# johannah/drqv2

Measured on AMD Instinct MI355X. Metric: agent updates/sec (batch=256, 9x84x84 obs), higher is better.
Workload: dtype f32; 1 GPU; cheetah_run batch_size=256/GPU (256 global) 9x84x84 u8 obs, A=6, feature_dim=50, hidden_dim=1024, fp32, use_tb=True; parallelism=dp1, global_batch=256

## Files before the change

drqv2_amd/_lib.py:

```python
import ctypes as C
import os

HERE = os.path.dirname(os.path.abspath(__file__))
LIB_PATH = os.path.join(HERE, "libdrqv2_hip.so")

c_float_p = C.c_void_p
c_u8_p = C.c_void_p
stream_t = C.c_void_p


class DrqStep(C.Structure):
    _fields_ = [
        ("B", C.c_int), ("global_B", C.c_int), ("C", C.c_int), ("A", C.c_int), ("F", C.c_int), ("H", C.c_int),
        ("obs", c_u8_p), ("next_obs", c_u8_p),
        ("action", c_float_p), ("reward", c_float_p), ("discount", c_float_p),
        ("shift_obs", c_float_p), ("shift_next", c_float_p),
        ("noise_critic", c_float_p), ("noise_actor", c_float_p),
        ("base_grid", c_float_p),
        ("params", c_float_p), ("grads", c_float_p), ("adam_m", c_float_p), ("adam_v", c_float_p),
        ("ws", c_float_p), ("ws_bytes", C.c_size_t),
        ("sums", c_float_p),
        ("lr", C.c_double), ("tau", C.c_double),
        ("std", C.c_float), ("clip", C.c_float),
        ("step_critic", C.c_long), ("step_enc", C.c_long), ("step_actor", C.c_long),
# ... 11 lines not shown

I, L, F, D, P, SZ = C.c_int, C.c_long, C.c_float, C.c_double, C.c_void_p, C.c_size_t

PROTOTYPES = {
    "drq_abi_version": (I, []),
    "drq_aug_fwd": (I, [P, P, P, P, I, I, I, I, I, P]),
    "drq_aug_fwd_f32": (I, [P, P, P, P, I, I, I, I, P]),
    "drq_conv1_aug_fwd": (I, [P, P, P, P, P, P, P, P, P, I, I, P]),
    "drq_conv1_aug_fwd_bf16": (I, [P, P, P, P, P, P, P, P, P, I, I, P]),
    "drq_conv1_aug_fwd_bf16_nhwc": (I, [P, P, P, P, P, P, P, P, P, I, I, P]),
    "drq_conv1_aug_fwd_indexed": (I, [P, P, P, P, P, P, P, P, P, P, P, I, I, P]),
    "drq_conv3x3_fwd": (I, [P, P, P, P, I, I, I, I, I, L, L, L, L, P]),
    "drq_conv3x3_dgrad": (I, [P, P, P, P, I, I, L, L, L, L, P]),
    "drq_conv3x3_fwd_wino": (I, [P, P, P, P, I, I, I, L, L, L, L, P]),
    "drq_conv3x3_dgrad_wino": (I, [P, P, P, P, I, I, L, L, L, L, P]),
    "drq_conv3x3_wgrad_wino": (I, [P, P, P, P, I, I, L, L, L, L, P, SZ, P]),
    "drq_conv3x3_wgrad": (I, [P, P, P, P, I, I, I, I, L, L, L, L, P, SZ, P]),
    "drq_conv3x3_wgrad_ws_bytes": (SZ, []),
    "drq_conv3x3_fwd_bf16": (I, [P, P, P, P, I, I, I, L, L, L, L, P]),
    "drq_conv3x3_dgrad_bf16": (I, [P, P, P, P, I, I, L, L, L, L, P]),
    "drq_conv3x3_wgrad_bf16": (I, [P, P, P, P, I, I, L, L, L, L, P, SZ, P]),
    "drq_conv3x3_fwd_bf16_nhwc": (I, [P, P, P, P, I, I, I, I, I, P]),
    "drq_conv3x3_dgrad_bf16_nhwc": (I, [P, P, P, P, I, I, I, I, L, L, L, L, P]),
    "drq_conv3x3_wgrad_bf16_nhwc": (I, [P, P, P, P, I, I, I, L, L, L, L, P, SZ, P]),
    "drq_gemm_f32": (I, [P, L, I, P, L, I, P, L, I, I, I, I, L, L, L, P, L, I, P, I, L, I, I, I, P, SZ, P]),
    "drq_gemm_batched_f32": (I, [I, P, L, I, P, L, I, P, L, I, I, I, P, I, P, I, P, I, I, I, P, SZ, P]),
    "drq_gemm_batched_bf16": (I, [I, P, L, I, P, L, I, P, L, I, I, I, P, I, P, I, P, I, I, P, SZ, P]),
    "drq_gemm_batched_partial": (I, [I, P, L, I, P, L, I, P, L, I, I, I, P, P, SZ, C.POINTER(I), P]),
    "drq_mlp_fwd": (I, [I, P, L, P, L, P, L, I, I, I, P, I, P, P, C.POINTER(I), P]),
    "drq_mlp_dgrad": (I, [I, P, L, P, L, P, L, I, I, I, P, I, P]),
# ... 29 lines not shown
    "drq_aug_bwd_f32": (I, [P, P, P, P, I, I, I, I, P]),
    "drq_tanh_bwd": (I, [P, P, P, L, P]),
    "drq_param_layout": (I, [I, I, I, I, C.POINTER(L), I]),
    "drq_step_ws_bytes": (SZ, [I, I, I, I, I]),
    "drq_step_ws_offset": (L, [I, I, I, I, I, I]),
    "drq_update_phase": (I, [C.POINTER(DrqStep), I]),
    "drq_update_phase_bc": (I, [C.POINTER(DrqStep), I, F]),
    "drq_act_forward": (I, [C.POINTER(DrqStep), P, I, P]),
    "drq_act_ws_bytes": (SZ, [I, I, I, I, I]),
    "drq_act_batch": (I, [P, I, I, I, I, P, I, P, F, P, P, P, SZ, P]),
    "drq_publish_sums": (I, [P, P, C.c_uint, P]),
    "drq_rng_draws": (I, [C.c_uint64, C.c_uint64, I, I, I, P, P, P, P, P]),
}

WS_IDS = ["AUG", "ACT1", "ACT2", "ACT3", "FEAT", "Z_NEXT", "Z_OBS", "HA_T", "HA_C", "H_AN", "H_AO", "Q", "TQ",
          "DQ", "MU_O", "DY4", "DY3", "DY2", "DY1", "DZ_C", "DZ_A", "HA_C2", "P1", "P2", "C1", "C2"]

PHASE_ALL, PHASE_CRITIC, PHASE_ACTOR, PHASE_OPT = -1, 0, 1, 2
PHASE_ENCODE, PHASE_CRITIC_HEADS, PHASE_CONV_BACKWARD, PHASE_ACTOR_FORWARD, PHASE_ACTOR_BACKWARD = 3, 4, 5, 6, 7
PHASE_ENCODER_OPT, PHASE_ACTOR_OPT = 8, 9
PHASE_CRITIC_OPT, PHASE_ACTOR_LOSS, PHASE_POLYAK, PHASE_REDRAW = 10, 11, 12, 13

_lib = None


class DrqError(RuntimeError):
    pass


def load():
    global _lib
# ... 41 lines not shown
```

drqv2_amd/csrc/conv_wino.hip:

```cpp
#include "common.h"
#include "internal.h"
#include "wino_u.h"
#include <type_traits>

namespace {

struct WinoArgs {
  const float* x;
  const float* w;
  const float* pre;
  const float* bias;
  const float* mask;
  float* y;
  int y_bs, y_cs, y_rs, y_off;
  unsigned x_bytes, y_bytes, mask_bytes;
  int nb;
  int relu;
  int wmode;
  int stagger;
};

typedef unsigned u32x4w __attribute__((ext_vector_type(4)));
typedef unsigned u32x2w __attribute__((ext_vector_type(2)));
typedef float f32x2w __attribute__((ext_vector_type(2)));

constexpr int kStagger = 0;

template <int HIN, bool MASK, bool RELU>
__global__ __launch_bounds__(256, 2) void conv3x3_wino_kernel(WinoArgs a) {
#pragma clang fp contract(off)
  constexpr int HOUT = HIN - 2;
  constexpr int TH = (HOUT + 1) / 2;
  constexpr int TT = TH * TH;
  constexpr int PLANE = HIN * HIN * 4;
  __shared__ __attribute__((aligned(16))) float U[16 * 8 * 64 * 2];

  const int tid = threadIdx.x;
  const int lane = tid & 63;
  const int wid = tid >> 6;
  const int tl = lane & 15;
  const int kk = lane >> 4;

  if (a.pre) {
// ... 12 lines not shown
  for (int h = 0; h < 2; ++h)
#pragma unroll
    for (int r = 0; r < 4; ++r) bv[h][r] = a.bias ? a.bias[16 * h + 4 * kk + r] : 0.f;
  __syncthreads();

  if (a.stagger) {
    const unsigned hwid = __builtin_amdgcn_s_getreg((4 << 0) | (0 << 6) | (31 << 11));
    if (hwid & 1u)
      for (int q = 0; q < a.stagger; ++q) __builtin_amdgcn_s_sleep(16);
  }

  const __amdgpu_buffer_rsrc_t xrs = __builtin_amdgcn_make_buffer_rsrc((void*)a.x, 0, a.x_bytes, 0x00020000);
  const __amdgpu_buffer_rsrc_t yrs = __builtin_amdgcn_make_buffer_rsrc((void*)a.y, 0, a.y_bytes, 0x00020000);
  const __amdgpu_buffer_rsrc_t mrs =
      __builtin_amdgcn_make_buffer_rsrc((void*)a.mask, 0, a.mask ? a.mask_bytes : 0, 0x00020000);
  constexpr int kDrop = (int)0x80000000u;

  const int ntile = a.nb * TT;
  const int nunit = (ntile + 15) >> 4;
  const int nwave = (int)gridDim.x * 4;
  const f32x2w* Ul = reinterpret_cast<const f32x2w*>(U) + lane;

  auto patch_voff = [&](int unit) {
    int t = unit * 16 + tl;
    t = t < ntile ? t : ntile - 1;
    const int b = t / TT, rem = t - b * TT;
    const int ty = rem / TH, tx = rem - ty * TH;
    return (((b * 32 + kk) * HIN + 2 * ty) * HIN + 2 * tx) * 4;
  };
  auto load_patch_row = [&](float (&d)[16], int voff, int c, int i) {
// ... 50 lines not shown
    const int t = valid ? t0 : ntile - 1;
    const int b = t / TT, rem = t - b * TT;
    const int ty = rem / TH, tx = rem - ty * TH;
    const bool c1ok = 2 * tx + 1 < HOUT, r1ok = 2 * ty + 1 < HOUT;
    const int ybase = (a.y_off + b * a.y_bs + (4 * kk) * a.y_cs + (2 * ty) * a.y_rs + 2 * tx) * 4;
    const int mbase = (((b * 32 + 4 * kk) * HOUT + 2 * ty) * HOUT + 2 * tx) * 4;
    int o64[2], o32[2];
#pragma unroll
    for (int i = 0; i < 2; ++i) {
      const bool rowok = valid && (i == 0 || r1ok);
      o64[i] = (rowok && c1ok) ? ybase : kDrop;
      o32[i] = (rowok && !c1ok) ? ybase : kDrop;
    }
    f32x4 acc[16][2];
    u32x2w mk[2][4][2];
#pragma unroll
    for (int c = 0; c < 8; ++c) {
      asm volatile("" ::: "memory");
      float t[16];
#pragma unroll
      for (int j = 0; j < 4; ++j) {
        t[0 * 4 + j] = d[0 * 4 + j] - d[2 * 4 + j];
        t[1 * 4 + j] = d[1 * 4 + j] + d[2 * 4 + j];
        t[2 * 4 + j] = d[2 * 4 + j] - d[1 * 4 + j];
        t[3 * 4 + j] = d[1 * 4 + j] - d[3 * 4 + j];
      }
      __builtin_amdgcn_sched_barrier(0);
      load_A(A1, c, 1);
      __builtin_amdgcn_sched_barrier(0);
      float V[16];
// ... 16 lines not shown
          const f32x2w Ap = A[p];
          if (c == 0) {
            const f32x4 z = {0.f, 0.f, 0.f, 0.f};
            const f32x4 b0 = {bv[0][0], bv[0][1], bv[0][2], bv[0][3]}, b1 = {bv[1][0], bv[1][1], bv[1][2], bv[1][3]};
            if constexpr (HSEL != 1) acc[pos][0] = __builtin_amdgcn_mfma_f32_16x16x4f32(Ap[0], V[pos], pos == 5 ? b0 : z, 0, 0, 0);
            if constexpr (HSEL != 0) acc[pos][1] = __builtin_amdgcn_mfma_f32_16x16x4f32(Ap[1], V[pos], pos == 5 ? b1 : z, 0, 0, 0);
          } else {
            if constexpr (HSEL != 1) acc[pos][0] = __builtin_amdgcn_mfma_f32_16x16x4f32(Ap[0], V[pos], acc[pos][0], 0, 0, 0);
            if constexpr (HSEL != 0) acc[pos][1] = __builtin_amdgcn_mfma_f32_16x16x4f32(Ap[1], V[pos], acc[pos][1], 0, 0, 0);
          }
        }
      };
      half_step(A0, 0);
      __builtin_amdgcn_sched_barrier(0);
      load_A(A0, (c + 1) & 7, 0);
      if constexpr (MASK) {
        if (c == 7) {
          constexpr int h0 = HSEL == 1 ? 1 : 0;
#pragma unroll
          for (int r = 0; r < 4; ++r)
#pragma unroll
            for (int i = 0; i < 2; ++i)
              mk[h0][r][i] = __builtin_amdgcn_raw_buffer_load_b64(mrs, mbase + i * (HOUT * 4),
                                                                  (16 * h0 + r) * (HOUT * HOUT * 4), 0);
        }
      }
      __builtin_amdgcn_sched_barrier(0);
      half_step(A1, 1);
      __builtin_amdgcn_sched_barrier(0);
    }
    {
      if constexpr (MASK && HSEL == 2) {
#pragma unroll
        for (int r = 0; r < 4; ++r)
#pragma unroll
          for (int i = 0; i < 2; ++i)
            mk[1][r][i] = __builtin_amdgcn_raw_buffer_load_b64(mrs, mbase + i * (HOUT * 4), (16 + r) * (HOUT * HOUT * 4), 0);
        __builtin_amdgcn_sched_barrier(0);
      }
      const int ycs4 = a.y_cs * 4, yrs4 = a.y_rs * 4;
#pragma unroll
      for (int h = (HSEL == 1 ? 1 : 0); h < (HSEL == 0 ? 1 : 2); ++h)
#pragma unroll
        for (int r = 0; r < 4; ++r) {
          float s[2][4];
#pragma unroll
          for (int j = 0; j < 4; ++j) {
            const float m0 = acc[0 * 4 + j][h][r], m1 = acc[1 * 4 + j][h][r], m2 = acc[2 * 4 + j][h][r],
                        m3 = acc[3 * 4 + j][h][r];
            s[0][j] = (m0 + m1) + m2;
            s[1][j] = (m1 - m2) - m3;
          }
          const int co = (16 * h + r);
#pragma unroll
          for (int i = 0; i < 2; ++i) {
            float y0 = (s[i][0] + s[i][1]) + s[i][2];
            float y1 = (s[i][1] - s[i][2]) - s[i][3];
            if constexpr (RELU) {
              y0 = __builtin_fmaxf(y0, 0.f);
              y1 = __builtin_fmaxf(y1, 0.f);
            }
            if constexpr (MASK) {
              const unsigned q0 = mk[h][r][i][0], q1 = mk[h][r][i][1];
              y0 = __uint_as_float(q0) > 0.f ? y0 : 0.f;
              y1 = __uint_as_float(q1) > 0.f ? y1 : 0.f;
            }
            const int soff = co * ycs4 + i * yrs4;
            const u32x2w pk = {__float_as_uint(y0), __float_as_uint(y1)};
            __builtin_amdgcn_raw_buffer_store_b64(pk, yrs, o64[i], soff, 0);
            __builtin_amdgcn_raw_buffer_store_b32(__float_as_uint(y0), yrs, o32[i], soff, 0);
          }
        }
    }
    voff = nvoff;
  };
  for (int i = 0; i < nfull; ++i) body(std::integral_constant<int, 2>{}, item_unit(i), item_unit(i + 1 < nitem ? i + 1 : i));
  if (has_half) {
    if (half_h == 0) body(std::integral_constant<int, 0>{}, half_unit, half_unit);
    else body(std::integral_constant<int, 1>{}, half_unit, half_unit);
  }
}

template <int HIN>
int launch_wino(const WinoArgs& a0, hipStream_t st) {
  WinoArgs a = a0;
  a.stagger = kStagger;
  constexpr int HOUT = HIN - 2, TH = (HOUT + 1) / 2;
  const long nunit = ((long)a.nb * TH * TH + 15) / 16;
  long blocks = (nunit + 3) / 4;
  const long cap = 2L * drq_num_cus();
  if (blocks > cap) blocks = cap;
  if (blocks < 1) blocks = 1;
  const dim3 g((unsigned)blocks), t(256);
  if (a.mask && a.relu) hipLaunchKernelGGL((conv3x3_wino_kernel<HIN, true, true>), g, t, 0, st, a);
  else if (a.mask) hipLaunchKernelGGL((conv3x3_wino_kernel<HIN, true, false>), g, t, 0, st, a);
  else if (a.relu) hipLaunchKernelGGL((conv3x3_wino_kernel<HIN, false, true>), g, t, 0, st, a);
  else hipLaunchKernelGGL((conv3x3_wino_kernel<HIN, false, false>), g, t, 0, st, a);
  DRQ_LAUNCH_CHECK();
  return DRQ_OK;
}

}

int drq_conv3x3_fwd_wino_pre(const float* x, const float* w, const float* u_image, const float* bias, float* y, int nb,
                             int hin, int relu, long y_bs, long y_cs, long y_rs, long y_off, hipStream_t st) {
  if (!x || !w || !y || nb <= 0) return DRQ_EARG;
  const size_t xb = (size_t)nb * 32 * hin * hin * 4;
  const size_t yb = (size_t)nb * y_bs * 4;
  if (xb >= (1ull << 31) || yb >= (1ull << 31) || y_off < 0 || y_bs <= 0) return DRQ_EARG;
  WinoArgs a{x, w, u_image, bias, nullptr, y, (int)y_bs, (int)y_cs, (int)y_rs, (int)y_off, (unsigned)xb, (unsigned)yb, 0u, nb, relu, 0, 0};
  if (hin == 41) return launch_wino<41>(a, st);
  if (hin == 39) return launch_wino<39>(a, st);
  if (hin == 37) return launch_wino<37>(a, st);
  return DRQ_EARG;
}

int drq_conv3x3_dgrad_wino_pre(const float* dy_pad, const float* w, const float* u_image, const float* mask, float* dx,
                               int nb, int hout, long dx_bs, long dx_cs, long dx_rs, long dx_off, hipStream_t st) {
  if (!dy_pad || !w || !dx || nb <= 0) return DRQ_EARG;
  const int hp = hout + 4;
  const size_t xb = (size_t)nb * 32 * hp * hp * 4;
  const size_t yb = (size_t)nb * dx_bs * 4;
  const size_t mb = (size_t)nb * 32 * (hout + 2) * (hout + 2) * 4;
  if (xb >= (1ull << 31) || yb >= (1ull << 31) || dx_off < 0 || dx_bs <= 0) return DRQ_EARG;
  WinoArgs a{dy_pad, w, u_image, nullptr, mask, dx, (int)dx_bs, (int)dx_cs, (int)dx_rs, (int)dx_off, (unsigned)xb, (unsigned)yb,
             (unsigned)mb, nb, 0, 1, 0};
  if (hp == 39) return launch_wino<39>(a, st);
  if (hp == 41) return launch_wino<41>(a, st);
  if (hp == 43) return launch_wino<43>(a, st);
  return DRQ_EARG;
}

DRQ_API int drq_conv3x3_fwd_wino(const float* x, const float* w, const float* bias, float* y, int nb, int hin, int relu,
                                 long y_bs, long y_cs, long y_rs, long y_off, hipStream_t st) {
  return drq_conv3x3_fwd_wino_pre(x, w, nullptr, bias, y, nb, hin, relu, y_bs, y_cs, y_rs, y_off, st);
}

DRQ_API int drq_conv3x3_dgrad_wino(const float* dy_pad, const float* w, const float* mask, float* dx, int nb, int hout,
                                   long dx_bs, long dx_cs, long dx_rs, long dx_off, hipStream_t st) {
  return drq_conv3x3_dgrad_wino_pre(dy_pad, w, nullptr, mask, dx, nb, hout, dx_bs, dx_cs, dx_rs, dx_off, st);
}
```

drqv2_amd/csrc/internal.h:

```cpp
#pragma once
#include "common.h"

int drq_ln_tanh_fwd_multi_ex(int n, const float* const* z, int ldz, const float* const* gamma,
                             const float* const* beta, float* const* out, const int* ldo, float* const* xhat,
                             float* const* rstd, int rows, int F, const float* const* tail, const int* tail_ld,
                             int tail_n, hipStream_t st);
int drq_ln_tanh_fwd_multi_part(int n, const float* const* z, int ldz, const float* const* gamma,
                               const float* const* beta, float* const* out, const int* ldo, float* const* xhat,
                               float* const* rstd, int rows, int F, const float* const* tail, const int* tail_ld,
                               int tail_n, const float* part, const float* const* bias, int splitk, hipStream_t st);
int drq_ln_tanh_bwd_part(const float* dh0, int ld0, const float* dh1, int ld1, const float* h, int ldh,
                         const float* xhat, const float* rstd, const float* gamma, float* dz, float* dln,
                         float* dgamma, float* dbeta, int rows, int F, const float* part, int splitk, int nprob,
                         int ldp, hipStream_t st);
int drq_ln_param_grad(const float* dln, const float* xhat, float* dgamma, float* dbeta, int rows, int F,
                      hipStream_t st);
int drq_qout_bwd_td(const float* tq1, const float* tq2, const float* q1, const float* q2, const float* reward,
                    const float* discount, float inv_global_B, float* sums, const float* const* h,
                    const float* const* w, float* const* dh, float* const* dw, float* const* db, int B, int H,
                    hipStream_t st);
int drq_qout_bwd_actor(const float* q1, const float* q2, const float* act, long lda, const float* mu, float std, int A,
                       float inv_global_B, float* sums, float* sums_host, unsigned seq, const float* const* h,
                       const float* const* w, float* const* dh, int B, int H, hipStream_t st);
int drq_policy_out_fwd(const float* h2, const float* w, const float* b, float* p3, int rows, int H, int A,
// ... 50 lines not shown
int drq_lnl1_fwd(int njobs, const float* const* part, const float* const* z, const float* const* bias,
                 const float* const* gamma, const float* const* beta, float* const* out, const int* ldo,
                 float* const* xhat, float* const* rstd, const float* const* tail, const int* tail_ld, const int* tail_n,
                 const int* rows, const int* nheads, const float* const* w, const float* const* b, float* const* y, int F,
                 int H, int splitk, long slab, hipStream_t st);
int drq_polout_l1_fwd(const float* p2, const float* w3, const float* b3, float* p3, int rows, int srow0, int H, int A,
                      int F, float std, float clip, int use_clip, const float* noise_hi, float* mu_hi, float* ha_hi,
                      long lda_hi, const float* noise_lo, float* mu_lo, float* ha_lo, long lda_lo, int nheads,
                      const float* const* w, const float* const* b, float* const* y, hipStream_t st);

int drq_conv1_aug_fwd_any(int bf_mma, const uint8_t* obs, const float* shift, const uint8_t* obs1, const float* shift1,
                          const float* base_grid, const float* w, const float* bias, float* xaug, float* y, int n,
                          int n_store, hipStream_t st, const float* const* wino_w, float* wino_u, const long* fidx0,
                          const long* fidx1);

int drq_conv3x3_fwd_wino_pre(const float* x, const float* w, const float* u_image, const float* bias, float* y, int nb,
                             int hin, int relu, long y_bs, long y_cs, long y_rs, long y_off, hipStream_t st);
int drq_conv3x3_dgrad_wino_pre(const float* dy_pad, const float* w, const float* u_image, const float* mask, float* dx,
                               int nb, int hout, long dx_bs, long dx_cs, long dx_rs, long dx_off, hipStream_t st);

int drq_conv3x3_fwd_bf16_lay(const void* x, const float* w, const float* bias, void* y, int nb, int hin, int relu,
                             long y_bs, long y_cs, long y_rs, long y_off, int lay, hipStream_t st);
int drq_conv3x3_dgrad_bf16_lay(const void* dy_pad, const float* w, const void* mask, void* dx, int nb, int hout,
                               long dx_bs, long dx_cs, long dx_rs, long dx_off, int lay, hipStream_t st);
int drq_conv3x3_wgrad_partial_bf16_lay(const void* x, const void* dy, int nb, int hin, long dy_bs, long dy_cs, long dy_rs,
                                       long dy_off, float* part, size_t part_bytes, int* nblocks, int lay,
                                       hipStream_t st);
int drq_conv3x3_wgrad_partial_bf16(const float* x, const float* dy, int nb, int hin, long dy_bs, long dy_cs, long dy_rs,
                                   long dy_off, float* part, size_t part_bytes, int* nblocks, hipStream_t st);

constexpr int kActMaxRows = 256;
struct ActWeights {
  const float *enc_w[4], *enc_b[4];
  const float *trunk_w, *trunk_b, *ln_g, *ln_b;
// ... 19 lines not shown
```

drqv2_amd/csrc/step.hip:

```cpp
#include "common.h"
#include "internal.h"
#include "../../include/drqv2_hip.h"

namespace {

constexpr long R = 32L * 35 * 35;
inline long al64(long x) { return (x + 63) & ~63L; }
inline long al512(long x) { return (x + 511) & ~511L; }

struct HeadOff {
  long trunk_w, trunk_b, ln_g, ln_b;
  long w[2][3], b[2][3];
};
enum { SEG_ENC, SEG_CRITIC, SEG_ACTOR, SEG_TARGET };
struct ParamLayout {
  long enc_w[4], enc_b[4];
  HeadOff critic, actor, target;
  long seg[8];
  long total;
  long flat[50];
  int nflat;
  long seg_beg(int net) const { return seg[2 * net]; }
  long seg_len(int net) const { return seg[2 * net + 1] - seg[2 * net]; }
};
// ... 47 lines not shown
}

struct WsLayout {
  long off[64];
  long total;
};
constexpr long kGemmWsFloats = 16L * 1024 * 1024;
enum {
  W_AUG = DRQ_WS_AUG, W_ACT1 = DRQ_WS_ACT1, W_ACT2 = DRQ_WS_ACT2, W_ACT3 = DRQ_WS_ACT3, W_FEAT = DRQ_WS_FEAT,
  W_Z_NEXT = DRQ_WS_Z_NEXT, W_Z_OBS = DRQ_WS_Z_OBS, W_HA_T = DRQ_WS_HA_T, W_HA_C = DRQ_WS_HA_C,
  W_H_AN = DRQ_WS_H_AN, W_H_AO = DRQ_WS_H_AO, W_Q = DRQ_WS_Q, W_TQ = DRQ_WS_TQ, W_DQ = DRQ_WS_DQ,
  W_MU_O = DRQ_WS_MU_O, W_DY4 = DRQ_WS_DY4, W_DY3 = DRQ_WS_DY3, W_DY2 = DRQ_WS_DY2, W_DY1 = DRQ_WS_DY1,
  W_DZ_C = DRQ_WS_DZ_C, W_DZ_A = DRQ_WS_DZ_A, W_HA_C2 = DRQ_WS_HA_C2,
  W_P1 = DRQ_WS_P1, W_P2 = DRQ_WS_P2,
  W_C1 = DRQ_WS_C1, W_C2 = DRQ_WS_C2,
  W_XHAT_C = DRQ_WS_NBUF_PUBLIC, W_RSTD_C, W_XHAT_A, W_RSTD_A, W_Z_C2,
  W_HROWS, W_P3, W_Z4,
  W_T1, W_T2,
  W_DC2, W_DC1, W_DHA, W_DLN, W_DPRE, W_DP2, W_DP1, W_DH_A, W_DA,
  W_GEMM_WS, W_CONV_WS,
  W_WINO_U,
  W_COUNT
};

WsLayout ws_layout(int B, int C, int A, int F, int H) {
  WsLayout w{};
  long off = 0;
  auto take = [&](int id, long n) {
    w.off[id] = off;
    off = al64(off + n);
// ... 35 lines not shown
  take(W_T2, 2L * B * H);
  take(W_C1, 2L * B * H);
  take(W_C2, 2L * B * H);
  take(W_DC2, 2L * B * H);
  take(W_DC1, 2L * B * H);
  take(W_DHA, 2L * B * (F + A));
  take(W_DLN, (long)B * F);
  take(W_DPRE, (long)B * A);
  take(W_DP2, (long)B * H);
  take(W_DP1, (long)B * H);
  take(W_DH_A, (long)B * F);
  take(W_DA, 2L * B * A);
  take(W_GEMM_WS, kGemmWsFloats);
  take(W_CONV_WS, (long)(drq_conv3x3_wgrad_ws_bytes() / sizeof(float)));
  take(W_WINO_U, 6L * 16384);
  w.total = off;
  return w;
}

#define CK(expr)                \
  do {                          \
    const int rc__ = (expr);    \
    if (rc__ != 0) return rc__; \
  } while (0)

struct Ctx {
  const DrqStep* s;
  ParamLayout P;
  WsLayout W;
  hipStream_t st;
  bool fuse_actor_loss = false;
  float bc_alpha = 0.f;
  bool bc() const { return bc_alpha > 0.f; }
  const float* a_beh() const { return ws(W_HA_C) + s->F; }
  float bc_scale() const { return 2.0f / ((float)s->global_B * (float)s->A); }
  bool qout_loss_fits_lds() const { return ((size_t)s->B + 5 * 1024 + 16) * 4 <= 60 * 1024; }
  bool actor_loss_fused() const { return fuse_actor_loss && qout_loss_fits_lds(); }
  bool fuse_rows() const {
    return !(s->flags & DRQ_STEP_NO_ROW_FUSION) && !s->bf16 && s->A <= 32 && s->F + s->A <= 64 && s->F % 2 == 0 &&
           s->A % 2 == 0 && s->H % 256 == 0;
  }
  bool use_gemm3() const { return !(s->flags & DRQ_STEP_NO_GEMM3) && !s->bf16; }
  int stamp(int idx) const {
    if (s->timing_events && idx < s->timing_n && hipEventRecord((hipEvent_t)s->timing_events[idx], st) != hipSuccess)
      return DRQ_EARG;
    return 0;
  }
  float* ws(int id) const { return s->ws + W.off[id]; }
  float* p(long off) const { return s->params + off; }
  float* g(long off) const { return s->grads + off; }
  int bf16() const { return s->bf16 ? 1 : 0; }
  bool acts16() const { return s->bf16 && !(s->flags & DRQ_STEP_BF16_FP32_ACTS); }
  bool grads16() const { return acts16() && !(s->flags & DRQ_STEP_BF16_FP32_GRADS); }
  int adam_segment(int net, long step, int target = -1) const {
    const long o = P.seg_beg(net);
    return drq_adam_flat(p(o), g(o), s->adam_m + o, s->adam_v + o, P.seg_len(net), s->lr, step, s->gscale,
                         target >= 0 ? p(P.seg_beg(target)) : nullptr, target >= 0 ? s->tau : 0.0, st);
// ... 41 lines not shown
    if (use_gemm3() && n >= 2) {
      const int rc = drq_gemm3_wgrad_dgrad(n, dy, lddy, x, ldx, dw, db, w, ldw, dx, lddx, mask, ldmask, Brows, N, K, st);
      if (rc != DRQ_EARG) return rc;
    }
    if (!bf16()) {
      const int rc = drq_gemm2_wgrad_dgrad(n, dy, lddy, x, ldx, dw, db, w, ldw, dx, lddx, mask, ldmask, Brows, N, K, st);
      if (rc != DRQ_EARG) return rc;
    }
    const int rc = wgrad(n, dy, lddy, x, ldx, dw, db, Brows, N, K);
    if (rc != 0) return rc;
    return dgrad(n, dy, lddy, w, ldw, dx, lddx, Brows, K, N, mask, ldmask);
  }
};

int encoder_forward(const Ctx& c, const float* x, int nb, float* a1, float* a2, float* a3, float* a4,
                    bool timed = false) {
  const ParamLayout& P = c.P;
  float* outs[4] = {a1, a2, a3, a4};
  const float* in = x ? x : a1;
  for (int l = x ? 0 : 1; l < 4; ++l) {
    const int hin = kEncH[l], hout = kEncH[l + 1];
    if (timed && l == 1) CK(c.stamp(0));
    if (c.bf16() && l > 0)
      CK(drq_conv3x3_fwd_bf16_lay(in, c.p(P.enc_w[l]), c.p(P.enc_b[l]), outs[l], nb, hin, 1, 32L * hout * hout,
                                  (long)hout * hout, hout, 0, (x == nullptr && c.acts16()) ? (l < 3 ? 3 : 1) : 0, c.st));
    else if (l > 0)
      CK(drq_conv3x3_fwd_wino_pre(in, c.p(P.enc_w[l]), x ? nullptr : c.ws(W_WINO_U) + (2L * (l - 1)) * 16384,
                                  c.p(P.enc_b[l]), outs[l], nb, hin, 1, 32L * hout * hout, (long)hout * hout, hout, 0,
                                  c.st));
    else
      CK(drq_conv3x3_fwd(in, c.p(P.enc_w[l]), c.p(P.enc_b[l]), outs[l], nb, l == 0 ? c.s->C : 32, hin, l == 0 ? 2 : 1,
                         1, 32L * hout * hout, (long)hout * hout, hout, 0, c.st));
    if (timed && l == 1) CK(c.stamp(1));
    in = outs[l];
  }
  return 0;
}

int policy_forward(const Ctx& c, const float* h, int rows, float* p1, float* p2, float* p3, int sample_from = -1,
                   const float* noise = nullptr, float* a_out = nullptr, long lda_out = 0,
                   const float* noise0 = nullptr, float* mu_out0 = nullptr, float* a_out0 = nullptr, long lda_out0 = 0,
                   bool* did_rows0 = nullptr) {
  const DrqStep* s = c.s;
  const HeadOff& a = c.P.actor;
// ... 41 lines not shown
    if (l == 2) CK(drq_qout_fwd(2 * nn, hh2, w, b, qq, B, H, c.st));
  }
  return 0;
}

int phase_encode(const Ctx& c) {
  const DrqStep* s = c.s;
  const int B = s->B;
  hipStream_t st = c.st;
  float* aug = c.ws(W_AUG);
  const float* wino_w[3] = {c.p(c.P.enc_w[1]), c.p(c.P.enc_w[2]), c.p(c.P.enc_w[3])};
  CK(drq_conv1_aug_fwd_any(c.acts16() ? 2 : c.bf16(), s->obs, s->shift_obs, s->next_obs, s->shift_next, s->base_grid,
                           c.p(c.P.enc_w[0]), c.p(c.P.enc_b[0]), aug, c.ws(W_ACT1), B, s->store_aug_next ? 2 * B : B, st,
                           c.bf16() ? nullptr : wino_w, c.bf16() ? nullptr : c.ws(W_WINO_U), s->obs_index,
                           s->next_obs_index));
  CK(encoder_forward(c, nullptr, 2 * B, c.ws(W_ACT1), c.ws(W_ACT2), c.ws(W_ACT3), c.ws(W_FEAT), true));
  return 0;
}

int phase_critic_heads(const Ctx& c) {
  const DrqStep* s = c.s;
  const ParamLayout& P = c.P;
  const int B = s->B, A = s->A, F = s->F, H = s->H, FA = F + A;
  hipStream_t st = c.st;
  float* feat = c.ws(W_FEAT);
  float* feat_obs = feat;
  float* feat_next = feat + (long)B * R;
  const HeadOff &cr = P.critic, &ac = P.actor, &tg = P.target;
  const long BH = (long)B * H;

  float* z4 = c.ws(W_Z4);
// ... 134 lines not shown
        CK(drq_conv3x3_wgrad_partial_bf16_lay(c.ws(actid[l]), dy, B, hin, 32L * hp * hp, (long)hp * hp, hp, 2L * hp + 2,
                                              part, quarter, &nblk[l],
                                              (c.acts16() ? 1 : 0) | (c.grads16() && l < 3 ? 2 : 0), st));
      else
        CK(drq_conv3x3_wgrad_partial(c.ws(actid[l]), dy, B, C, hin, 2, 32L * hp * hp, (long)hp * hp, hp, 2L * hp + 2,
                                     part, quarter, &nblk[l], st));
    }
    if (l >= 1) {
      const int hpi = hin + 4;
      if (l == 2) CK(c.stamp(2));
      if (c.bf16())
        CK(drq_conv3x3_dgrad_bf16_lay(dy, c.p(P.enc_w[l]), c.ws(actid[l]), c.ws(dyid[l - 1]), B, hout, 32L * hpi * hpi,
                                      (long)hpi * hpi, hpi, 2L * hpi + 2,
                                      (c.acts16() ? 4 : 0) | (c.grads16() && l < 3 ? 1 : 0) | (c.grads16() && l > 1 ? 2 : 0),
                                      st));
      else
        CK(drq_conv3x3_dgrad_wino_pre(dy, c.p(P.enc_w[l]), c.ws(W_WINO_U) + (2L * (l - 1) + 1) * 16384, c.ws(actid[l]),
                                      c.ws(dyid[l - 1]), B, hout, 32L * hpi * hpi, (long)hpi * hpi, hpi, 2L * hpi + 2,
                                      st));
      if (l == 2) CK(c.stamp(3));
    }
  }
  if (merged) {
    const float *xs[3], *dys[3];
    float* ps[3];
    long bs[3], cs[3], rs[3], off[3];
    for (int k = 0; k < 3; ++k) {
      const int l = k + 1, hp = kEncH[l + 1] + 4;
      xs[k] = c.ws(actid[l]); dys[k] = c.ws(dyid[l]); ps[k] = const_cast<float*>(parts[l]);
      bs[k] = 32L * hp * hp; cs[k] = (long)hp * hp; rs[k] = hp; off[k] = 2L * hp + 2;
// ... 314 lines not shown
```

drqv2_amd/ops.py:

```python
import torch

from . import _lib
from ._lib import check, ptr

ENC_H = (84, 41, 39, 37, 35)


def _alloc(shape, dtype, device, kind="out"):
    if kind == "zero":
        return torch.zeros(shape, device=device, dtype=dtype)
    return torch.empty(shape, device=device, dtype=dtype)


def _stream():
    return torch.cuda.current_stream().cuda_stream


def _need(t, dtype=torch.float32, name="tensor"):
    if not (isinstance(t, torch.Tensor) and t.is_cuda):
        raise _lib.DrqError(f"{name}: a GPU tensor is required (the HIP path has no CPU fallback)")
    if t.device.index != torch.cuda.current_device():
        raise _lib.DrqError(f"{name} lives on {t.device} but the current device is cuda:{torch.cuda.current_device()}: "
                            "wrap the call in torch.cuda.device(...)")
    if t.dtype != dtype or not t.is_contiguous():
# ... 108 lines not shown
        return dx
    dx = _alloc((nb, 32, hin, hin), torch.float32, dy_pad.device)
    if wino:
        check(lib.drq_conv3x3_dgrad_wino(ptr(dy_pad), ptr(w), ptr(mask), ptr(dx), nb, hout, 32 * hin * hin, hin * hin, hin,
                                         0, _stream()), "drq_conv3x3_dgrad_wino")
        return dx
    if bf16:
        check(lib.drq_conv3x3_dgrad_bf16(ptr(dy_pad), ptr(w), ptr(mask), ptr(dx), nb, hout, 32 * hin * hin, hin * hin, hin,
                                         0, _stream()), "drq_conv3x3_dgrad_bf16")
        return dx
    check(lib.drq_conv3x3_dgrad(ptr(dy_pad), ptr(w), ptr(mask), ptr(dx), nb, hout, 32 * hin * hin, hin * hin, hin, 0,
                                _stream()), "drq_conv3x3_dgrad")
    return dx


def conv3x3_wgrad(x, dy, stride, bf16=False, wino=False, ws=None):
    lib = _lib.load()
    _need(x, name="x")
    if not (dy.is_cuda and dy.dtype == torch.float32 and dy.stride(3) == 1):
        raise _lib.DrqError("dy: GPU fp32 with unit innermost stride required")
    nb, cin, hin, _ = x.shape
    dw = _alloc((32, cin, 3, 3), torch.float32, x.device)
    db = _alloc((32,), torch.float32, x.device)
    nbytes = lib.drq_conv3x3_wgrad_ws_bytes()
    if ws is None:
        ws = _alloc((nbytes // 4,), torch.float32, x.device, "ws")
    elif ws.numel() * 4 < nbytes:
        raise _lib.DrqError("conv3x3_wgrad: workspace too small")
    if wino:
        check(lib.drq_conv3x3_wgrad_wino(ptr(x), dy.data_ptr(), ptr(dw), ptr(db), nb, hin, dy.stride(0), dy.stride(1),
# ... 364 lines not shown
```

include/drqv2_hip.h:

```cpp
#ifndef DRQV2_HIP_H
#define DRQV2_HIP_H
#include <stddef.h>
#include <stdint.h>

#ifdef __cplusplus
extern "C" {
#endif

typedef void* drq_stream_t;

#define DRQ_OK 0
#define DRQ_EARG (-1)
#define DRQ_EWS (-2)

int drq_abi_version(void);

int drq_aug_fwd(const uint8_t* obs, const float* shift_xy, const float* base_grid, float* out, int n, int c,
                int hw, int pad, int fuse_norm, drq_stream_t stream);
int drq_aug_fwd_f32(const float* x, const float* shift_xy, const float* base_grid, float* out, int n, int c,
                    int hw, int pad, drq_stream_t stream);

int drq_conv1_aug_fwd(const uint8_t* obs, const float* shift, const uint8_t* obs1, const float* shift1,
                      const float* base_grid, const float* w, const float* bias, float* xaug, float* y, int n,
                      int n_store, drq_stream_t stream);
// ... 3 lines not shown
int drq_conv1_aug_fwd_bf16(const uint8_t* obs, const float* shift, const uint8_t* obs1, const float* shift1,
                           const float* base_grid, const float* w, const float* bias, float* xaug, float* y, int n,
                           int n_store, drq_stream_t stream);
int drq_conv1_aug_fwd_bf16_nhwc(const uint8_t* obs, const float* shift, const uint8_t* obs1, const float* shift1,
                                const float* base_grid, const float* w, const float* bias, float* xaug, void* y_nhwc,
                                int n, int n_store, drq_stream_t stream);

int drq_conv3x3_fwd(const float* x, const float* w, const float* bias, float* y, int nb, int cin, int hin,
                    int stride, int relu, long y_bs, long y_cs, long y_rs, long y_off, drq_stream_t stream);
int drq_conv3x3_dgrad(const float* dy_pad, const float* w, const float* mask, float* dx, int nb, int hout,
                      long dx_bs, long dx_cs, long dx_rs, long dx_off, drq_stream_t stream);
int drq_conv3x3_fwd_wino(const float* x, const float* w, const float* bias, float* y, int nb, int hin, int relu,
                         long y_bs, long y_cs, long y_rs, long y_off, drq_stream_t stream);
int drq_conv3x3_dgrad_wino(const float* dy_pad, const float* w, const float* mask, float* dx, int nb, int hout,
                           long dx_bs, long dx_cs, long dx_rs, long dx_off, drq_stream_t stream);
int drq_conv3x3_wgrad_wino(const float* x, const float* dy, float* dw, float* db, int nb, int hin, long dy_bs,
                           long dy_cs, long dy_rs, long dy_off, float* ws, size_t ws_bytes, drq_stream_t stream);
int drq_conv3x3_wgrad(const float* x, const float* dy, float* dw, float* db, int nb, int cin, int hin,
                      int stride, long dy_bs, long dy_cs, long dy_rs, long dy_off, float* ws, size_t ws_bytes,
                      drq_stream_t stream);
size_t drq_conv3x3_wgrad_ws_bytes(void);

int drq_conv3x3_fwd_bf16(const float* x, const float* w, const float* bias, float* y, int nb, int hin, int relu,
                         long y_bs, long y_cs, long y_rs, long y_off, drq_stream_t stream);
int drq_conv3x3_dgrad_bf16(const float* dy_pad, const float* w, const float* mask, float* dx, int nb, int hout,
                           long dx_bs, long dx_cs, long dx_rs, long dx_off, drq_stream_t stream);
int drq_conv3x3_wgrad_bf16(const float* x, const float* dy, float* dw, float* db, int nb, int hin, long dy_bs,
                           long dy_cs, long dy_rs, long dy_off, float* ws, size_t ws_bytes, drq_stream_t stream);
int drq_conv3x3_fwd_bf16_nhwc(const void* x, const float* w, const float* bias, void* y, int nb, int hin, int relu,
                              int x_nhwc, int y_nhwc, drq_stream_t stream);
// ... 138 lines not shown
  float gscale;
  drq_stream_t stream;
  float* sums_host;
  int store_aug_next;
  int bf16;
  void* const* timing_events;
  int timing_n;
  const int64_t* obs_index;
  const int64_t* next_obs_index;
  int flags;
} DrqStep;
#define DRQ_STEP_NO_ROW_FUSION 1
#define DRQ_STEP_NO_GEMM3 2
#define DRQ_STEP_BF16_FP32_ACTS 4
#define DRQ_STEP_BF16_FP32_GRADS 8

int drq_param_layout(int C, int A, int F, int H, long* out, int cap);
#define DRQ_PARAM_LAYOUT_LEN 59

size_t drq_step_ws_bytes(int B, int C, int A, int F, int H);
long drq_step_ws_offset(int B, int C, int A, int F, int H, int buffer_id);
enum {
  DRQ_WS_AUG = 0, DRQ_WS_ACT1, DRQ_WS_ACT2, DRQ_WS_ACT3, DRQ_WS_FEAT, DRQ_WS_Z_NEXT, DRQ_WS_Z_OBS,
  DRQ_WS_HA_T, DRQ_WS_HA_C, DRQ_WS_H_AN, DRQ_WS_H_AO, DRQ_WS_Q, DRQ_WS_TQ, DRQ_WS_DQ, DRQ_WS_MU_O,
  DRQ_WS_DY4, DRQ_WS_DY3, DRQ_WS_DY2, DRQ_WS_DY1, DRQ_WS_DZ_C, DRQ_WS_DZ_A, DRQ_WS_HA_C2,
  DRQ_WS_P1, DRQ_WS_P2,
  DRQ_WS_C1, DRQ_WS_C2,
  DRQ_WS_NBUF_PUBLIC
};

enum {
  DRQ_PHASE_ALL = -1, DRQ_PHASE_CRITIC = 0, DRQ_PHASE_ACTOR = 1, DRQ_PHASE_OPT = 2,
  DRQ_PHASE_ENCODE = 3, DRQ_PHASE_CRITIC_HEADS = 4, DRQ_PHASE_CONV_BACKWARD = 5, DRQ_PHASE_ACTOR_FORWARD = 6,
  DRQ_PHASE_ACTOR_BACKWARD = 7, DRQ_PHASE_ENCODER_OPT = 8, DRQ_PHASE_ACTOR_OPT = 9,
  DRQ_PHASE_CRITIC_OPT = 10, DRQ_PHASE_ACTOR_LOSS = 11, DRQ_PHASE_POLYAK = 12, DRQ_PHASE_REDRAW = 13
};
int drq_update_phase(const DrqStep* s, int phase);
int drq_update_phase_bc(const DrqStep* s, int phase, float bc_alpha);

int drq_publish_sums(const float* sums, float* sums_host, unsigned seq, drq_stream_t stream);

int drq_act_forward(const DrqStep* s, const uint8_t* obs, int n, float* mu_out);
// ... 10 lines not shown
```

Measured before the change: 991.3 updates/s.

## Pack encoder ReLU masks into bits for Winograd conv backward

The forward Winograd conv kernels for encoder layers 2 and 3 now emit a packed bitmask of positive ReLU outputs for the first B frames. The dgrad kernels read that bitmask instead of the fp32 activation tensor to mask gradients. This replaces a full fp32 activation read in the backward pass with a much smaller bit read, at the cost of extra stores in the forward pass, new workspace buffers and new kernel variants.

```diff
diff --git a/drqv2_amd/_lib.py b/drqv2_amd/_lib.py
--- a/drqv2_amd/_lib.py
+++ b/drqv2_amd/_lib.py
@@ -49,6 +49,9 @@
     "drq_conv3x3_dgrad": (I, [P, P, P, P, I, I, L, L, L, L, P]),
     "drq_conv3x3_fwd_wino": (I, [P, P, P, P, I, I, I, L, L, L, L, P]),
     "drq_conv3x3_dgrad_wino": (I, [P, P, P, P, I, I, L, L, L, L, P]),
+    "drq_relu_bits_nbytes": (SZ, [I, I]),
+    "drq_conv3x3_fwd_wino_bits": (I, [P, P, P, P, P, I, I, I, L, L, L, L, P]),
+    "drq_conv3x3_dgrad_wino_bits": (I, [P, P, P, P, I, I, L, L, L, L, P]),
     "drq_conv3x3_wgrad_wino": (I, [P, P, P, P, I, I, L, L, L, L, P, SZ, P]),
     "drq_conv3x3_wgrad": (I, [P, P, P, P, I, I, I, I, L, L, L, L, P, SZ, P]),
     "drq_conv3x3_wgrad_ws_bytes": (SZ, []),
@@ -108,7 +111,7 @@
 }
 
 WS_IDS = ["AUG", "ACT1", "ACT2", "ACT3", "FEAT", "Z_NEXT", "Z_OBS", "HA_T", "HA_C", "H_AN", "H_AO", "Q", "TQ",
-          "DQ", "MU_O", "DY4", "DY3", "DY2", "DY1", "DZ_C", "DZ_A", "HA_C2", "P1", "P2", "C1", "C2"]
+          "DQ", "MU_O", "DY4", "DY3", "DY2", "DY1", "DZ_C", "DZ_A", "HA_C2", "P1", "P2", "C1", "C2", "BITS2", "BITS3"]
 
 PHASE_ALL, PHASE_CRITIC, PHASE_ACTOR, PHASE_OPT = -1, 0, 1, 2
 PHASE_ENCODE, PHASE_CRITIC_HEADS, PHASE_CONV_BACKWARD, PHASE_ACTOR_FORWARD, PHASE_ACTOR_BACKWARD = 3, 4, 5, 6, 7
diff --git a/drqv2_amd/csrc/conv_wino.hip b/drqv2_amd/csrc/conv_wino.hip
--- a/drqv2_amd/csrc/conv_wino.hip
+++ b/drqv2_amd/csrc/conv_wino.hip
@@ -18,6 +18,8 @@
   int relu;
   int wmode;
   int stagger;
+  unsigned* bits;
+  unsigned bits_bytes;
 };
 
 typedef unsigned u32x4w __attribute__((ext_vector_type(4)));
@@ -26,7 +28,7 @@
 
 constexpr int kStagger = 0;
 
-template <int HIN, bool MASK, bool RELU>
+template <int HIN, bool MASK, bool RELU, int BITS = 0>
 __global__ __launch_bounds__(256, 2) void conv3x3_wino_kernel(WinoArgs a) {
 #pragma clang fp contract(off)
   constexpr int HOUT = HIN - 2;
@@ -69,6 +71,8 @@
   const __amdgpu_buffer_rsrc_t yrs = __builtin_amdgcn_make_buffer_rsrc((void*)a.y, 0, a.y_bytes, 0x00020000);
   const __amdgpu_buffer_rsrc_t mrs =
       __builtin_amdgcn_make_buffer_rsrc((void*)a.mask, 0, a.mask ? a.mask_bytes : 0, 0x00020000);
+  const __amdgpu_buffer_rsrc_t brs =
+      __builtin_amdgcn_make_buffer_rsrc((void*)a.bits, 0, (BITS && a.bits) ? a.bits_bytes : 0, 0x00020000);
   constexpr int kDrop = (int)0x80000000u;
 
   const int ntile = a.nb * TT;
@@ -149,6 +153,8 @@
     }
     f32x4 acc[16][2];
     u32x2w mk[2][4][2];
+    unsigned bw = 0;
+    auto boff = [&] { return (unit * 64 + (int)(threadIdx.x & 63)) * 4; };
 #pragma unroll
     for (int c = 0; c < 8; ++c) {
       asm volatile("" ::: "memory");
@@ -195,7 +201,12 @@
       half_step(A0, 0);
       __builtin_amdgcn_sched_barrier(0);
       load_A(A0, (c + 1) & 7, 0);
-      if constexpr (MASK) {
+      if constexpr (MASK && BITS == 2) {
+        if (c == 7) {
+          if constexpr (HSEL == 2) bw = __builtin_amdgcn_raw_buffer_load_b32(brs, boff(), 0, 0);
+          else bw = (unsigned)__builtin_amdgcn_raw_buffer_load_b16(brs, boff() + 2 * HSEL, 0, 0) << (16 * HSEL);
+        }
+      } else if constexpr (MASK) {
         if (c == 7) {
           constexpr int h0 = HSEL == 1 ? 1 : 0;
 #pragma unroll
@@ -211,7 +222,7 @@
       __builtin_amdgcn_sched_barrier(0);
     }
     {
-      if constexpr (MASK && HSEL == 2) {
+      if constexpr (MASK && BITS != 2 && HSEL == 2) {
 #pragma unroll
         for (int r = 0; r < 4; ++r)
 #pragma unroll
@@ -241,7 +252,14 @@
               y0 = __builtin_fmaxf(y0, 0.f);
               y1 = __builtin_fmaxf(y1, 0.f);
             }
-            if constexpr (MASK) {
+            if constexpr (BITS == 1) {
+              bw |= (y0 > 0.f ? 1u : 0u) << (16 * h + 4 * r + 2 * i);
+              bw |= (y1 > 0.f ? 2u : 0u) << (16 * h + 4 * r + 2 * i);
+            }
+            if constexpr (MASK && BITS == 2) {
+              y0 = (bw >> (16 * h + 4 * r + 2 * i)) & 1u ? y0 : 0.f;
+              y1 = (bw >> (16 * h + 4 * r + 2 * i)) & 2u ? y1 : 0.f;
+            } else if constexpr (MASK) {
               const unsigned q0 = mk[h][r][i][0], q1 = mk[h][r][i][1];
               y0 = __uint_as_float(q0) > 0.f ? y0 : 0.f;
               y1 = __uint_as_float(q1) > 0.f ? y1 : 0.f;
@@ -251,7 +269,12 @@
             __builtin_amdgcn_raw_buffer_store_b64(pk, yrs, o64[i], soff, 0);
             __builtin_amdgcn_raw_buffer_store_b32(__float_as_uint(y0), yrs, o32[i], soff, 0);
           }
+          if constexpr (BITS == 1) __builtin_amdgcn_sched_barrier(0);
         }
+      if constexpr (BITS == 1) {
+        if constexpr (HSEL == 2) __builtin_amdgcn_raw_buffer_store_b32(bw, brs, boff(), 0, 0);
+        else __builtin_amdgcn_raw_buffer_store_b16((unsigned short)(bw >> (16 * HSEL)), brs, boff() + 2 * HSEL, 0, 0);
+      }
     }
     voff = nvoff;
   };
@@ -273,6 +296,22 @@
   if (blocks > cap) blocks = cap;
   if (blocks < 1) blocks = 1;
   const dim3 g((unsigned)blocks), t(256);
+  if constexpr (HIN == 41 || HIN == 39) {
+    if (a.bits && a.wmode == 0) {
+      if (!a.relu || a.mask) return DRQ_EARG;
+      hipLaunchKernelGGL((conv3x3_wino_kernel<HIN, false, true, 1>), g, t, 0, st, a);
+      DRQ_LAUNCH_CHECK();
+      return DRQ_OK;
+    }
+  }
+  if constexpr (HIN == 41 || HIN == 39) {
+    if (a.bits && a.wmode == 1) {
+      hipLaunchKernelGGL((conv3x3_wino_kernel<HIN, true, false, 2>), g, t, 0, st, a);
+      DRQ_LAUNCH_CHECK();
+      return DRQ_OK;
+    }
+  }
+  if (a.bits) return DRQ_EARG;
   if (a.mask && a.relu) hipLaunchKernelGGL((conv3x3_wino_kernel<HIN, true, true>), g, t, 0, st, a);
   else if (a.mask) hipLaunchKernelGGL((conv3x3_wino_kernel<HIN, true, false>), g, t, 0, st, a);
   else if (a.relu) hipLaunchKernelGGL((conv3x3_wino_kernel<HIN, false, true>), g, t, 0, st, a);
@@ -284,12 +323,15 @@
 }
 
 int drq_conv3x3_fwd_wino_pre(const float* x, const float* w, const float* u_image, const float* bias, float* y, int nb,
-                             int hin, int relu, long y_bs, long y_cs, long y_rs, long y_off, hipStream_t st) {
+                             int hin, int relu, long y_bs, long y_cs, long y_rs, long y_off, hipStream_t st,
+                             unsigned* bits, int n_bits_frames) {
   if (!x || !w || !y || nb <= 0) return DRQ_EARG;
+  if (bits && (n_bits_frames <= 0 || n_bits_frames > nb || !relu)) return DRQ_EARG;
   const size_t xb = (size_t)nb * 32 * hin * hin * 4;
   const size_t yb = (size_t)nb * y_bs * 4;
   if (xb >= (1ull << 31) || yb >= (1ull << 31) || y_off < 0 || y_bs <= 0) return DRQ_EARG;
-  WinoArgs a{x, w, u_image, bias, nullptr, y, (int)y_bs, (int)y_cs, (int)y_rs, (int)y_off, (unsigned)xb, (unsigned)yb, 0u, nb, relu, 0, 0};
+  WinoArgs a{x, w, u_image, bias, nullptr, y, (int)y_bs, (int)y_cs, (int)y_rs, (int)y_off, (unsigned)xb, (unsigned)yb, 0u, nb, relu, 0, 0,
+             bits, bits ? (unsigned)drq_relu_bits_bytes(n_bits_frames, hin - 2) : 0u};
   if (hin == 41) return launch_wino<41>(a, st);
   if (hin == 39) return launch_wino<39>(a, st);
   if (hin == 37) return launch_wino<37>(a, st);
@@ -297,27 +339,50 @@
 }
 
 int drq_conv3x3_dgrad_wino_pre(const float* dy_pad, const float* w, const float* u_image, const float* mask, float* dx,
-                               int nb, int hout, long dx_bs, long dx_cs, long dx_rs, long dx_off, hipStream_t st) {
+                               int nb, int hout, long dx_bs, long dx_cs, long dx_rs, long dx_off, hipStream_t st,
+                               const unsigned* bits) {
   if (!dy_pad || !w || !dx || nb <= 0) return DRQ_EARG;
+  if (bits && mask) return DRQ_EARG;
   const int hp = hout + 4;
   const size_t xb = (size_t)nb * 32 * hp * hp * 4;
   const size_t yb = (size_t)nb * dx_bs * 4;
   const size_t mb = (size_t)nb * 32 * (hout + 2) * (hout + 2) * 4;
   if (xb >= (1ull << 31) || yb >= (1ull << 31) || dx_off < 0 || dx_bs <= 0) return DRQ_EARG;
   WinoArgs a{dy_pad, w, u_image, nullptr, mask, dx, (int)dx_bs, (int)dx_cs, (int)dx_rs, (int)dx_off, (unsigned)xb, (unsigned)yb,
-             (unsigned)mb, nb, 0, 1, 0};
+             (unsigned)mb, nb, 0, 1, 0, const_cast<unsigned*>(bits),
+             bits ? (unsigned)drq_relu_bits_bytes(nb, hout + 2) : 0u};
   if (hp == 39) return launch_wino<39>(a, st);
   if (hp == 41) return launch_wino<41>(a, st);
   if (hp == 43) return launch_wino<43>(a, st);
   return DRQ_EARG;
 }
 
+size_t drq_relu_bits_bytes(int nb, int h) {
+  const long th = (h + 1) / 2;
+  return (size_t)(((long)nb * th * th + 15) / 16) * 256;
+}
+
 DRQ_API int drq_conv3x3_fwd_wino(const float* x, const float* w, const float* bias, float* y, int nb, int hin, int relu,
                                  long y_bs, long y_cs, long y_rs, long y_off, hipStream_t st) {
   return drq_conv3x3_fwd_wino_pre(x, w, nullptr, bias, y, nb, hin, relu, y_bs, y_cs, y_rs, y_off, st);
 }
 
+DRQ_API int drq_conv3x3_fwd_wino_bits(const float* x, const float* w, const float* bias, float* y, uint32_t* bits,
+                                      int n_bits_frames, int nb, int hin, long y_bs, long y_cs, long y_rs, long y_off,
+                                      hipStream_t st) {
+  if (!bits) return DRQ_EARG;
+  return drq_conv3x3_fwd_wino_pre(x, w, nullptr, bias, y, nb, hin, 1, y_bs, y_cs, y_rs, y_off, st, bits, n_bits_frames);
+}
+
 DRQ_API int drq_conv3x3_dgrad_wino(const float* dy_pad, const float* w, const float* mask, float* dx, int nb, int hout,
                                    long dx_bs, long dx_cs, long dx_rs, long dx_off, hipStream_t st) {
   return drq_conv3x3_dgrad_wino_pre(dy_pad, w, nullptr, mask, dx, nb, hout, dx_bs, dx_cs, dx_rs, dx_off, st);
 }
+
+DRQ_API int drq_conv3x3_dgrad_wino_bits(const float* dy_pad, const float* w, const uint32_t* bits, float* dx, int nb,
+                                        int hout, long dx_bs, long dx_cs, long dx_rs, long dx_off, hipStream_t st) {
+  if (!bits) return DRQ_EARG;
+  return drq_conv3x3_dgrad_wino_pre(dy_pad, w, nullptr, nullptr, dx, nb, hout, dx_bs, dx_cs, dx_rs, dx_off, st, bits);
+}
+
+DRQ_API size_t drq_relu_bits_nbytes(int nb, int h) { return (nb > 0 && h > 0) ? drq_relu_bits_bytes(nb, h) : 0; }
diff --git a/drqv2_amd/csrc/internal.h b/drqv2_amd/csrc/internal.h
--- a/drqv2_amd/csrc/internal.h
+++ b/drqv2_amd/csrc/internal.h
@@ -88,10 +88,13 @@
                           int n_store, hipStream_t st, const float* const* wino_w, float* wino_u, const long* fidx0,
                           const long* fidx1);
 
+size_t drq_relu_bits_bytes(int nb, int h);
 int drq_conv3x3_fwd_wino_pre(const float* x, const float* w, const float* u_image, const float* bias, float* y, int nb,
-                             int hin, int relu, long y_bs, long y_cs, long y_rs, long y_off, hipStream_t st);
+                             int hin, int relu, long y_bs, long y_cs, long y_rs, long y_off, hipStream_t st,
+                             unsigned* bits = nullptr, int n_bits_frames = 0);
 int drq_conv3x3_dgrad_wino_pre(const float* dy_pad, const float* w, const float* u_image, const float* mask, float* dx,
-                               int nb, int hout, long dx_bs, long dx_cs, long dx_rs, long dx_off, hipStream_t st);
+                               int nb, int hout, long dx_bs, long dx_cs, long dx_rs, long dx_off, hipStream_t st,
+                               const unsigned* bits = nullptr);
 
 int drq_conv3x3_fwd_bf16_lay(const void* x, const float* w, const float* bias, void* y, int nb, int hin, int relu,
                              long y_bs, long y_cs, long y_rs, long y_off, int lay, hipStream_t st);
diff --git a/drqv2_amd/csrc/step.hip b/drqv2_amd/csrc/step.hip
--- a/drqv2_amd/csrc/step.hip
+++ b/drqv2_amd/csrc/step.hip
@@ -85,6 +85,7 @@
   W_DZ_C = DRQ_WS_DZ_C, W_DZ_A = DRQ_WS_DZ_A, W_HA_C2 = DRQ_WS_HA_C2,
   W_P1 = DRQ_WS_P1, W_P2 = DRQ_WS_P2,
   W_C1 = DRQ_WS_C1, W_C2 = DRQ_WS_C2,
+  W_BITS2 = DRQ_WS_BITS2, W_BITS3 = DRQ_WS_BITS3,
   W_XHAT_C = DRQ_WS_NBUF_PUBLIC, W_RSTD_C, W_XHAT_A, W_RSTD_A, W_Z_C2,
   W_HROWS, W_P3, W_Z4,
   W_T1, W_T2,
@@ -150,6 +151,8 @@
   take(W_GEMM_WS, kGemmWsFloats);
   take(W_CONV_WS, (long)(drq_conv3x3_wgrad_ws_bytes() / sizeof(float)));
   take(W_WINO_U, 6L * 16384);
+  take(W_BITS2, (long)(drq_relu_bits_bytes(B, 39) / sizeof(float)));
+  take(W_BITS3, (long)(drq_relu_bits_bytes(B, 37) / sizeof(float)));
   w.total = off;
   return w;
 }
@@ -177,6 +180,8 @@
            s->A % 2 == 0 && s->H % 256 == 0;
   }
   bool use_gemm3() const { return !(s->flags & DRQ_STEP_NO_GEMM3) && !s->bf16; }
+  bool relu_bits_on() const { return !s->bf16 && !(s->flags & DRQ_STEP_FP32_RELU_MASKS); }
+  unsigned* relu_bits(int layer) const { return reinterpret_cast<unsigned*>(ws(W_BITS2 + (layer - 1))); }
   int stamp(int idx) const {
     if (s->timing_events && idx < s->timing_n && hipEventRecord((hipEvent_t)s->timing_events[idx], st) != hipSuccess)
       return DRQ_EARG;
@@ -248,7 +253,7 @@
 };
 
 int encoder_forward(const Ctx& c, const float* x, int nb, float* a1, float* a2, float* a3, float* a4,
-                    bool timed = false) {
+                    bool timed = false, int n_bits_frames = 0) {
   const ParamLayout& P = c.P;
   float* outs[4] = {a1, a2, a3, a4};
   const float* in = x ? x : a1;
@@ -261,7 +266,7 @@
     else if (l > 0)
       CK(drq_conv3x3_fwd_wino_pre(in, c.p(P.enc_w[l]), x ? nullptr : c.ws(W_WINO_U) + (2L * (l - 1)) * 16384,
                                   c.p(P.enc_b[l]), outs[l], nb, hin, 1, 32L * hout * hout, (long)hout * hout, hout, 0,
-                                  c.st));
+                                  c.st, (n_bits_frames > 0 && l < 3) ? c.relu_bits(l) : nullptr, l < 3 ? n_bits_frames : 0));
     else
       CK(drq_conv3x3_fwd(in, c.p(P.enc_w[l]), c.p(P.enc_b[l]), outs[l], nb, l == 0 ? c.s->C : 32, hin, l == 0 ? 2 : 1,
                          1, 32L * hout * hout, (long)hout * hout, hout, 0, c.st));
@@ -333,7 +338,8 @@
                            c.p(c.P.enc_w[0]), c.p(c.P.enc_b[0]), aug, c.ws(W_ACT1), B, s->store_aug_next ? 2 * B : B, st,
                            c.bf16() ? nullptr : wino_w, c.bf16() ? nullptr : c.ws(W_WINO_U), s->obs_index,
                            s->next_obs_index));
-  CK(encoder_forward(c, nullptr, 2 * B, c.ws(W_ACT1), c.ws(W_ACT2), c.ws(W_ACT3), c.ws(W_FEAT), true));
+  CK(encoder_forward(c, nullptr, 2 * B, c.ws(W_ACT1), c.ws(W_ACT2), c.ws(W_ACT3), c.ws(W_FEAT), true,
+                     c.relu_bits_on() ? B : 0));
   return 0;
 }
 
@@ -498,6 +504,10 @@
                                       (long)hpi * hpi, hpi, 2L * hpi + 2,
                                       (c.acts16() ? 4 : 0) | (c.grads16() && l < 3 ? 1 : 0) | (c.grads16() && l > 1 ? 2 : 0),
                                       st));
+      else if (l >= 2 && c.relu_bits_on())
+        CK(drq_conv3x3_dgrad_wino_pre(dy, c.p(P.enc_w[l]), c.ws(W_WINO_U) + (2L * (l - 1) + 1) * 16384, nullptr,
+                                      c.ws(dyid[l - 1]), B, hout, 32L * hpi * hpi, (long)hpi * hpi, hpi, 2L * hpi + 2,
+                                      st, c.relu_bits(l - 1)));
       else
         CK(drq_conv3x3_dgrad_wino_pre(dy, c.p(P.enc_w[l]), c.ws(W_WINO_U) + (2L * (l - 1) + 1) * 16384, c.ws(actid[l]),
                                       c.ws(dyid[l - 1]), B, hout, 32L * hpi * hpi, (long)hpi * hpi, hpi, 2L * hpi + 2,
diff --git a/drqv2_amd/ops.py b/drqv2_amd/ops.py
--- a/drqv2_amd/ops.py
+++ b/drqv2_amd/ops.py
@@ -146,6 +146,38 @@
     return dx
 
 
+def relu_bits_words(nb, h):
+    return _lib.load().drq_relu_bits_nbytes(nb, h) // 4
+
+
+def conv3x3_fwd_wino_bits(x, w, b, n_bits_frames=None):
+    lib = _lib.load()
+    _need(x, name="x"), _need(w, name="w"), _need(b, name="b")
+    nb, _, hin, _ = x.shape
+    hout = hin - 2
+    nbf = nb if n_bits_frames is None else n_bits_frames
+    y = _alloc((nb, 32, hout, hout), torch.float32, x.device)
+    bits = _alloc((relu_bits_words(nbf, hout),), torch.int32, x.device)
+    check(lib.drq_conv3x3_fwd_wino_bits(ptr(x), ptr(w), ptr(b), ptr(y), ptr(bits), nbf, nb, hin, 32 * hout * hout,
+                                        hout * hout, hout, 0, _stream()), "drq_conv3x3_fwd_wino_bits")
+    return y, bits
+
+
+def conv3x3_dgrad_wino_bits(dy_pad, w, bits, pad_out=False):
+    lib = _lib.load()
+    _need(dy_pad, name="dy_pad"), _need(w, name="w"), _need(bits, torch.int32, "bits")
+    nb, _, hp, _ = dy_pad.shape
+    hout = hp - 4
+    hin = hout + 2
+    if bits.numel() < relu_bits_words(nb, hin):
+        raise _lib.DrqError("conv3x3_dgrad_wino_bits: the bit buffer is too small")
+    hpi = hin + 4 if pad_out else hin
+    dx = _alloc((nb, 32, hpi, hpi), torch.float32, dy_pad.device, "zero" if pad_out else "out")
+    check(lib.drq_conv3x3_dgrad_wino_bits(ptr(dy_pad), ptr(w), ptr(bits), ptr(dx), nb, hout, 32 * hpi * hpi, hpi * hpi, hpi,
+                                          2 * hpi + 2 if pad_out else 0, _stream()), "drq_conv3x3_dgrad_wino_bits")
+    return dx
+
+
 def conv3x3_wgrad(x, dy, stride, bf16=False, wino=False, ws=None):
     lib = _lib.load()
     _need(x, name="x")
diff --git a/include/drqv2_hip.h b/include/drqv2_hip.h
--- a/include/drqv2_hip.h
+++ b/include/drqv2_hip.h
@@ -41,6 +41,12 @@
                          long y_bs, long y_cs, long y_rs, long y_off, drq_stream_t stream);
 int drq_conv3x3_dgrad_wino(const float* dy_pad, const float* w, const float* mask, float* dx, int nb, int hout,
                            long dx_bs, long dx_cs, long dx_rs, long dx_off, drq_stream_t stream);
+size_t drq_relu_bits_nbytes(int nb, int h);
+int drq_conv3x3_fwd_wino_bits(const float* x, const float* w, const float* bias, float* y, uint32_t* bits,
+                              int n_bits_frames, int nb, int hin, long y_bs, long y_cs, long y_rs, long y_off,
+                              drq_stream_t stream);
+int drq_conv3x3_dgrad_wino_bits(const float* dy_pad, const float* w, const uint32_t* bits, float* dx, int nb, int hout,
+                                long dx_bs, long dx_cs, long dx_rs, long dx_off, drq_stream_t stream);
 int drq_conv3x3_wgrad_wino(const float* x, const float* dy, float* dw, float* db, int nb, int hin, long dy_bs,
                            long dy_cs, long dy_rs, long dy_off, float* ws, size_t ws_bytes, drq_stream_t stream);
 int drq_conv3x3_wgrad(const float* x, const float* dy, float* dw, float* db, int nb, int cin, int hin,
@@ -209,6 +215,7 @@
 #define DRQ_STEP_NO_GEMM3 2
 #define DRQ_STEP_BF16_FP32_ACTS 4
 #define DRQ_STEP_BF16_FP32_GRADS 8
+#define DRQ_STEP_FP32_RELU_MASKS 16
 
 int drq_param_layout(int C, int A, int F, int H, long* out, int cap);
 #define DRQ_PARAM_LAYOUT_LEN 59
@@ -221,6 +228,7 @@
   DRQ_WS_DY4, DRQ_WS_DY3, DRQ_WS_DY2, DRQ_WS_DY1, DRQ_WS_DZ_C, DRQ_WS_DZ_A, DRQ_WS_HA_C2,
   DRQ_WS_P1, DRQ_WS_P2,
   DRQ_WS_C1, DRQ_WS_C2,
+  DRQ_WS_BITS2, DRQ_WS_BITS3,
   DRQ_WS_NBUF_PUBLIC
 };
 
```

After: 986.7 updates/s. Within noise of the previous version (-0.5%).
